# EndMy5uffering/4DGaussianSplatRendering

Hardware: AMD Instinct MI355X
Metric: Gaussians/sec + ms/frame @1080p; sort permutation bit-exact (higher is better)
Workload: dtype f32; 1 GPU; 1,000,000 random 3D splats in a 400^3 cube, single 1080p frame (BASELINE.json configs[1]); splats=1000000, width=1920, height=1080, sort=on, frame_lanes=4, tile_list_entries=1377553, longest_tile_list=477, unordered_draws=3158, staged_list_draws=3158, overflow_reruns=3, depth_sort_passes=3, record_bytes_read_by_projection=64, tiles_composited=14400, tiles=32400, key_index_buffer_pairs=4, lane_streams_rejected_at_create=1

## Files before the change

### 4dgaussiansplatrendering_amd/csrc/gs4d_internal.h

```cpp
#pragma once
#include <hip/hip_runtime.h>
#include <stdint.h>
#include <stddef.h>
#include <string>
#include <vector>
#include "../../include/gs4d.h"

namespace gs4d {

constexpr int TILE = 8;
constexpr int PROJ_FLOATS = 16;


enum class Outputs : int { Colour = 0, Aux = 1, Ids = 2 };
constexpr bool has_aux(Outputs o) { return o >= Outputs::Aux; }
constexpr bool has_ids(Outputs o) { return o >= Outputs::Ids; }
static_assert(sizeof(gs4d_record_stat) == 16 && offsetof(gs4d_record_stat, wsum) == 8, "the 64-bit sum is naturally aligned in a 16-byte record");
struct StatOut { gs4d_record_stat* rec = nullptr; uint32_t n = 0; };
struct Target {
    float4* fb; uint32_t* tstate; uint32_t epoch; float4 clear;
    Outputs out; float2* aux; uint32_t* ids;
    const float* z = nullptr;
    StatOut stats;
};
// ... 182 lines not shown
    TRect r{ tx0, ty0, wx, ty1 - ty0 + 1u, 1u, 0u };
    if (shard_world > 1u) {
        const uint32_t first = r.ty0 + (shard_rank + shard_world - r.ty0 % shard_world) % shard_world;
        r.rows = first > ty1 ? 0u : (ty1 - first) / shard_world + 1u;
        r.ty0 = first; r.tstep = shard_world;
    }
    r.count = r.wx * r.rows;
    return r;
}
__device__ __forceinline__ TRect tile_rect(uint32_t rect0, uint32_t rect1, uint32_t shard_rank, uint32_t shard_world) {
    const uint32_t x0 = rect0 & 0xFFFFu, y0 = rect0 >> 16, x1 = rect1 & 0xFFFFu, y1 = rect1 >> 16;
    if (x0 > x1 || y0 > y1) return TRect{ 0u, 0u, 0u, 0u, 1u, 0u };
    return tile_rect_of(x0 / TILE, y0 / TILE, x1 / TILE - x0 / TILE + 1u, y1 / TILE, shard_rank, shard_world);
}
constexpr uint32_t TRECT_NONE = 0xFFFFFFFFu, TRECT_WIDE = 0xFFFFFFFEu;
__device__ __forceinline__ uint32_t pack_trect(uint32_t rect0, uint32_t rect1) {
    const uint32_t x0 = rect0 & 0xFFFFu, y0 = rect0 >> 16, x1 = rect1 & 0xFFFFu, y1 = rect1 >> 16;
    if (x0 > x1 || y0 > y1) return TRECT_NONE;
    const uint32_t tx0 = x0 / TILE, ty0 = y0 / TILE, wx = x1 / TILE - tx0, wy = y1 / TILE - ty0;
    if (tx0 >= 1023u || ty0 >= 1023u || wx >= 63u || wy >= 63u) return TRECT_WIDE;
    return tx0 | (ty0 << 10) | (wx << 20) | (wy << 26);
}
__device__ __forceinline__ TRect unpack_trect(uint32_t w, const float4* __restrict__ proj, uint32_t rec, uint32_t shard_rank, uint32_t shard_world) {
    if (w == TRECT_NONE) return TRect{ 0u, 0u, 0u, 0u, 1u, 0u };
    if (w == TRECT_WIDE) { const float4 c = proj[(size_t)rec * 4 + 2]; return tile_rect(__float_as_uint(c.z), __float_as_uint(c.w), shard_rank, shard_world); }
    const uint32_t tx0 = w & 1023u, ty0 = (w >> 10) & 1023u;
    return tile_rect_of(tx0, ty0, ((w >> 20) & 63u) + 1u, ty0 + (w >> 26), shard_rank, shard_world);
}
__device__ __forceinline__ uint32_t tile_of(const TRect& r, uint32_t j, uint32_t tiles_x) { return (r.ty0 + (j / r.wx) * r.tstep) * tiles_x + r.tx0 + j % r.wx; }
template <class F> __device__ __forceinline__ void for_each_tile(const TRect& r, uint32_t tiles_x, F f) {
    uint32_t rowbase = r.ty0 * tiles_x + r.tx0;
    for (uint32_t y = 0; y < r.rows; ++y) { for (uint32_t x = 0; x < r.wx; ++x) f(rowbase + x); rowbase += r.tstep * tiles_x; }
}
#endif

hipError_t launch_soa_repack(hipStream_t st, const float* aos96, size_t n, float4* soa , uint32_t* bbox , const SoaInfo& info);
inline const float4* soa_sig3(const float4* soa, size_t n, const SoaInfo& info) { return info.layout == SOA_STATIC3D ? nullptr : soa + (info.layout == SOA_SYM ? 3 : 5) * n; }
struct PreOut { float4* proj; uint32_t* trects; bool aux = false; };
hipError_t launch_preprocess_4d(hipStream_t st, const float4* soa, size_t soa_n , const SoaInfo& info, size_t n, const Uniforms& u, int W, int H, PreOut out, const TileCount& tc);
hipError_t launch_preprocess_3d(hipStream_t st, const float* verts72, size_t n, const Uniforms& u, int W, int H, PreOut out, const TileCount& tc);
hipError_t launch_preprocess_2d(hipStream_t st, const float* rec48, size_t n, const Uniforms& u, int W, int H, PreOut out, const TileCount& tc);

struct BinScratch {
    uint32_t* total = nullptr;
    uint32_t* ranges = nullptr; size_t tiles_cap = 0;
    unsigned long long* status = nullptr; size_t block_cap = 0;
    uint32_t epoch = 0;
    uint32_t ticket_base = 0;
};
hipError_t bin_scratch_reserve(hipStream_t st, BinScratch& b, size_t ninst, size_t ntiles);
void bin_scratch_free(BinScratch& b);
hipError_t launch_binning(hipStream_t st, BinScratch& b, const uint32_t* trects, bool trects_in_order, const float4* proj, const uint32_t* order, uint32_t* order_copy, size_t ninst, size_t nrecords, int tiles_x, int tiles_y,
                          uint32_t* pair_keys, uint32_t* pair_vals, size_t pair_cap, uint32_t* err, uint32_t* ghist, int passes, uint32_t* total_host, int shard_rank, int shard_world);
hipError_t launch_tile_ranges(hipStream_t st, BinScratch& b, const uint32_t* pair_keys, size_t pair_cap, size_t ntiles);

hipError_t launch_composite(hipStream_t st, const float4* proj, const uint32_t* pair_vals, uint32_t* ranges, const uint32_t* total, int tiles_x, int tiles_y,
                            int W, int H, int premult_c, const Target& t, int blend_src, int blend_dst, uint32_t draw_ord);
hipError_t launch_fill_unwritten(hipStream_t st, const Target& t, int tiles_x, int tiles_y, int W, int H);
hipError_t launch_pack_rgba8(hipStream_t st, const float4* fb, const uint32_t* tstate, uint32_t epoch, const float clear[4], int W, int H, int tiles_x, uint32_t* out);
hipError_t launch_pack_rgba8_band(hipStream_t st, const float4* fb, const uint32_t* tstate, uint32_t epoch, const float clear[4], int W, int H, int tiles_x, int rank, int world, int band_rows, uint32_t* out);

struct LineParams { float vp[16]; float rgba[4]; int W, H; int blend_src, blend_dst; };
hipError_t launch_lines(hipStream_t st, const float* verts_dev, size_t nverts, int dims, int strip, const LineParams& p, float width, uint32_t* cnt, float4* fb);

constexpr uint32_t COMPACT_TILE = 2048;
struct KeepRule { uint32_t min_pixels, min_wmax; uint64_t min_wsum; uint32_t invert; };
// ... 97 lines not shown
```

### 4dgaussiansplatrendering_amd/csrc/preprocess.hip

```cpp
#include "gs4d_internal.h"
#include <algorithm>
#include <cstdlib>

namespace gs4d {

__device__ __forceinline__ uint32_t f2ord(float f) { const uint32_t u = __float_as_uint(f); return (u & 0x80000000u) ? ~u : (u | 0x80000000u); }

struct SoaConsts { float v[8]; };
template <int LAYOUT>
__global__ __launch_bounds__(256) void k_soa_repack(const float4* __restrict__ aos, uint32_t n, float4* __restrict__ soa, uint32_t* __restrict__ bbox, SoaConsts cs) {
    constexpr bool COMPACT = LAYOUT != SOA_FULL;
    __shared__ float4 stage[4][384];
    __shared__ uint32_t red[4][16];
    const uint32_t lane = threadIdx.x & 63u, w = threadIdx.x >> 6;
    uint32_t lo[7], hi[7];
#pragma unroll
    for (int k = 0; k < 7; ++k) { lo[k] = 0xFFFFFFFFu; hi[k] = 0u; }
    bool bad = false, asym = false;
    for (uint32_t chunk = blockIdx.x; chunk * 256u < n; chunk += gridDim.x) {
        const uint32_t rec0 = (chunk * 4u + w) * 64u;
        const uint32_t nrec = rec0 < n ? min(64u, n - rec0) : 0u;
#pragma unroll
        for (int j = 0; j < 6; ++j) {
            uint32_t f = j * 64u + lane;
// ... 32 lines not shown
        __builtin_amdgcn_wave_barrier();
    }
#pragma unroll
    for (int k = 0; k < 7; ++k) {
#pragma unroll
        for (int off = 32; off > 0; off >>= 1) { lo[k] = min(lo[k], (uint32_t)__shfl_xor(lo[k], off, 64)); hi[k] = max(hi[k], (uint32_t)__shfl_xor(hi[k], off, 64)); }
    }
    const bool anybad = __ballot(bad) != 0ull;
    if (COMPACT && __ballot(asym) != 0ull && lane == 0) atomicOr(&bbox[15], 1u);
    if (lane == 0) {
#pragma unroll
        for (int k = 0; k < 7; ++k) { red[w][k] = lo[k]; red[w][7 + k] = hi[k]; }
        red[w][14] = anybad ? 1u : 0u;
    }
    __syncthreads();
    if (threadIdx.x < 15u) {
        const uint32_t k = threadIdx.x;
        uint32_t v = red[0][k];
        for (int ww = 1; ww < 4; ++ww) v = k < 7u ? min(v, red[ww][k]) : k < 14u ? max(v, red[ww][k]) : (v | red[ww][k]);
        if (k < 7u) atomicMin(&bbox[k], v); else if (k < 14u) atomicMax(&bbox[k], v); else if (v) atomicOr(&bbox[14], 1u);
    }
}

hipError_t launch_soa_repack(hipStream_t st, const float* aos96, size_t n, float4* soa, uint32_t* bbox, const SoaInfo& info) {
    if (n == 0) return hipSuccess;
    const unsigned blocks = (unsigned)std::min<size_t>((n + 255) / 256, 2048);
    SoaConsts cs; for (int k = 0; k < 8; ++k) cs.v[k] = info.consts[k];
    if (info.layout == SOA_STATIC3D) k_soa_repack<SOA_STATIC3D><<<dim3(blocks), dim3(256), 0, st>>>((const float4*)aos96, (uint32_t)n, soa, bbox, cs);
    else if (info.layout == SOA_SYM) k_soa_repack<SOA_SYM><<<dim3(blocks), dim3(256), 0, st>>>((const float4*)aos96, (uint32_t)n, soa, bbox, cs);
    else k_soa_repack<SOA_FULL><<<dim3(blocks), dim3(256), 0, st>>>((const float4*)aos96, (uint32_t)n, soa, bbox, cs);
    return hipGetLastError();
}

struct PU { float V[16]; float P[16]; float time, min_opacity; int W, H; };

__device__ __forceinline__ float maxf_glsl(float a, float b) { return a >= b ? a : b; }
__device__ __forceinline__ void normalize2(float& x, float& y) { float tx = x * x, ty = y * y; float s = 1.0f / sqrtf(tx + ty); x = x * s; y = y * s; }

struct Quad { float e0x, e0y, e1x, e1y, s0, s1; };

__device__ __forceinline__ void eigen2(float u00, float u01, float u10, float u11, bool guard, float& lx, float& ly, Quad& q) {
    float m = (u00 + u11) * 0.5f;
    float p = (u00 * u11) - (u01 * u10);
    float d = sqrtf((m * m) - p);
    lx = maxf_glsl(m - d, 0.000001f);
    ly = maxf_glsl(m + d, 0.000001f);
    float ax, ay, bx, by;
    if (guard && u01 == 0.0f) { ax = 1.0f; ay = 0.0f; bx = 0.0f; by = 1.0f; }
    else {
        ax = u01; ay = lx - u00;
        normalize2(ax, ay);
        bx = ay; by = -ax;
        normalize2(ax, ay); normalize2(bx, by);
    }
    normalize2(ax, ay); normalize2(bx, by);
    q.e0x = ax; q.e0y = ay; q.e1x = bx; q.e1y = by;
}

__device__ __forceinline__ bool fin(float x) { return isfinite(x); }

__device__ __forceinline__ uint2 emit(const PreOut& out, uint32_t i, bool valid, const Quad& q, float ncx, float ncy, float kx, float ky,
                                      int W, int H, float r, float g, float b, float alpha, bool clamp_rgb, float depth) {
    float cx = 0, cy = 0, a0x = 0, a0y = 0, a1x = 0, a1y = 0, hx = 0, hy = 0;
    uint32_t rect0 = 1u, rect1 = 0u;
    if (valid) {
        float hw = (float)W * 0.5f, hh = (float)H * 0.5f;
        float sx = kx * hw, sy = ky * hh;
        cx = fmaf(ncx, hw, hw);
        cy = fmaf(ncy, hh, hh);
        float r0 = 1.0f / q.s0, r1 = 1.0f / q.s1;
        a0x = (q.e0x * r0) / sx; a0y = (q.e0y * r0) / sy;
        a1x = (q.e1x * r1) / sx; a1y = (q.e1y * r1) / sy;
        hx = 0.5f * (fabsf(q.e0x) * q.s0 + fabsf(q.e1x) * q.s1) * fabsf(sx);
        hy = 0.5f * (fabsf(q.e0y) * q.s0 + fabsf(q.e1y) * q.s1) * fabsf(sy);
        valid = fin(cx) && fin(cy) && fin(a0x) && fin(a0y) && fin(a1x) && fin(a1y) && fin(hx) && fin(hy) && fin(alpha);
        if (valid) {
            float mx = 0.01f + 1e-5f * hx, my = 0.01f + 1e-5f * hy;
            float fx0 = ceilf(cx - hx - mx - 0.5f), fx1 = floorf(cx + hx + mx - 0.5f);
            float fy0 = ceilf(cy - hy - my - 0.5f), fy1 = floorf(cy + hy + my - 0.5f);
            fx0 = fmaxf(fx0, 0.0f); fy0 = fmaxf(fy0, 0.0f);
            fx1 = fminf(fx1, (float)(W - 1)); fy1 = fminf(fy1, (float)(H - 1));
            if (fx0 <= fx1 && fy0 <= fy1) {
                rect0 = (uint32_t)fx0 | ((uint32_t)fy0 << 16);
                rect1 = (uint32_t)fx1 | ((uint32_t)fy1 << 16);
            }
        }
    }
    if (!valid) { cx = cy = a0x = a0y = a1x = a1y = hx = hy = 0.0f; alpha = 0.0f; rect0 = 1u; rect1 = 0u; depth = 0.0f; }
    if (clamp_rgb) { r = fminf(fmaxf(r, 0.0f), 1.0f); g = fminf(fmaxf(g, 0.0f), 1.0f); b = fminf(fmaxf(b, 0.0f), 1.0f); }
    if (out.trects) out.trects[i] = pack_trect(rect0, rect1);
    float4* o = out.proj + (size_t)i * 4;
    o[0] = make_float4(cx, cy, a0x, a1x);
    o[1] = make_float4(a0y, a1y, r, g);
    o[2] = make_float4(b, alpha, __uint_as_float(rect0), __uint_as_float(rect1));
    o[3] = make_float4(hx, hy, valid ? 1.0f : 0.0f, out.aux ? depth : 0.0f);
    return make_uint2(rect0, rect1);
}

__device__ __forceinline__ void count_buckets(uint32_t* h, uint32_t nbm, uint32_t tiles_x, const TRect& r) {
    const bool big = r.count > 16u;
    if (!big) for_each_tile(r, tiles_x, [&](uint32_t t) { atomicAdd(&h[t & nbm], 1u); });
    uint64_t m = __ballot(big);
    const uint32_t lane = threadIdx.x & 63u;
    while (m) {
        const int src = __ffsll((long long)m) - 1;
        m &= m - 1ull;
        TRect rr;
        rr.tx0 = __shfl(r.tx0, src, 64); rr.ty0 = __shfl(r.ty0, src, 64); rr.wx = __shfl(r.wx, src, 64);
        rr.rows = __shfl(r.rows, src, 64); rr.tstep = __shfl(r.tstep, src, 64); rr.count = __shfl(r.count, src, 64);
        for (uint32_t j = lane; j < rr.count; j += 64u) atomicAdd(&h[tile_of(rr, j, tiles_x) & nbm], 1u);
    }
}

__device__ __forceinline__ void place_buckets(uint32_t* cur, uint32_t nbm, uint32_t nbs, uint32_t tiles_x, const TRect& r, uint32_t key, uint32_t rec, uint2* stage) {
    const bool big = r.count > 16u;
    if (!big) for_each_tile(r, tiles_x, [&](uint32_t t) { stage[atomicAdd(&cur[t & nbm], 1u)] = make_uint2(key, ((t >> nbs) << 24) | rec); });
    uint64_t m = __ballot(big);
    const uint32_t lane = threadIdx.x & 63u;
    while (m) {
        const int src = __ffsll((long long)m) - 1;
        m &= m - 1ull;
        TRect rr;
        rr.tx0 = __shfl(r.tx0, src, 64); rr.ty0 = __shfl(r.ty0, src, 64); rr.wx = __shfl(r.wx, src, 64);
        rr.rows = __shfl(r.rows, src, 64); rr.tstep = __shfl(r.tstep, src, 64); rr.count = __shfl(r.count, src, 64);
        const uint32_t key2 = __shfl(key, src, 64), rec2 = __shfl(rec, src, 64);
        for (uint32_t j = lane; j < rr.count; j += 64u) { const uint32_t t = tile_of(rr, j, tiles_x); stage[atomicAdd(&cur[t & nbm], 1u)] = make_uint2(key2, ((t >> nbs) << 24) | rec2); }
    }
}

__device__ __forceinline__ uint32_t blend_key_4d(const KeySrc& ks, uint32_t i, const float4& p, const float4& s) {
    if (ks.mode == KEYSRC_INDEX) return i;
    float key;
    if (ks.mode == KEYSRC_REF) {
        float ct = ks.t - p.w;
        float x = p.x + s.x * ct;
        float y = p.y + s.y * ct;
        float z = p.z + s.z * ct;
        float dx = x - ks.camx, dy = y - ks.camy, dz = z - ks.camz;
        key = 1.0f / sqrtf(dx * dx + dy * dy + dz * dz);
    } else {
        float k = (1.0f / s.w) * (ks.t - p.w);
        float x = p.x + k * s.x, y = p.y + k * s.y, z = p.z + k * s.z;
        float zv = ((ks.vr0 * x + ks.vr1 * y) + ks.vr2 * z) + ks.vr3;
        key = 1.0f / fmaxf(-zv, 1e-20f);
    }
    return __float_as_uint(key) - ks.bias;
}

__device__ __forceinline__ bool project3d(const PU& u, float mx, float my, float mz, const float C[3][3], Quad& q, float& ncx, float& ncy, float& depth) {
// ... 24 lines not shown
    float T[3][3], Tt[3][3], A[3][3], cov[3][3];
#pragma unroll
    for (int c = 0; c < 3; ++c)
#pragma unroll
        for (int r = 0; r < 3; ++r) T[c][r] = Wt[0][r] * J[c][0] + Wt[1][r] * J[c][1] + Wt[2][r] * J[c][2];
#pragma unroll
    for (int c = 0; c < 3; ++c)
#pragma unroll
        for (int r = 0; r < 3; ++r) Tt[c][r] = T[r][c];
#pragma unroll
    for (int c = 0; c < 3; ++c)
#pragma unroll
        for (int r = 0; r < 3; ++r) A[c][r] = Tt[0][r] * C[c][0] + Tt[1][r] * C[c][1] + Tt[2][r] * C[c][2];
#pragma unroll
    for (int c = 0; c < 2; ++c)
#pragma unroll
        for (int r = 0; r < 2; ++r) cov[c][r] = A[0][r] * T[c][0] + A[1][r] * T[c][1] + A[2][r] * T[c][2];
    float lx, ly;
    eigen2(cov[0][0], cov[0][1], cov[1][0], cov[1][1], false, lx, ly, q);
    q.s0 = sqrtf(lx); q.s1 = sqrtf(ly);
    ncx = psx; ncy = psy;
    return true;
}

struct Src4D { const float4* soa; uint32_t stride; };
struct Src4DSym { const float4* soa; uint32_t stride; };
struct Src4DStatic { const float4* soa; uint32_t stride; SoaConsts cs; };
struct Src3D { const float* verts; };
struct Src2D { const float* recs; };

__device__ __forceinline__ uint2 project_4d(const float4& pos, const float4& col, const float4& s0, const float4& s1, const float4& s2, const float4& s3,
                                            uint32_t i, const PU& u, const PreOut& out, const KeySrc& ks, uint32_t& key);
__device__ __forceinline__ uint2 project_record(const Src4D& src, uint32_t n, uint32_t i, const PU& u, const PreOut& out, const KeySrc& ks, uint32_t& key) {
    const float4* __restrict__ soa = src.soa;
    const size_t ps = src.stride;
    const float4 pos = soa[i], col = soa[ps + i];
    const float4 s0 = soa[2 * ps + i], s1 = soa[3 * ps + i], s2 = soa[4 * ps + i], s3 = soa[5 * ps + i];
    return project_4d(pos, col, s0, s1, s2, s3, i, u, out, ks, key);
}
__device__ __forceinline__ uint2 project_record(const Src4DSym& src, uint32_t n, uint32_t i, const PU& u, const PreOut& out, const KeySrc& ks, uint32_t& key) {
    const float4* __restrict__ soa = src.soa;
    const size_t ps = src.stride;
    const float4 pos = soa[i], col = soa[ps + i], U = soa[2 * ps + i], V = soa[3 * ps + i];
    const float2 W = reinterpret_cast<const float2*>(soa + 4 * ps)[i];
    return project_4d(pos, col, make_float4(U.x, U.y, U.z, V.x), make_float4(U.y, U.w, W.x, V.y), make_float4(U.z, W.x, W.y, V.z), V, i, u, out, ks, key);
}
__device__ __forceinline__ uint2 project_record(const Src4DStatic& src, uint32_t n, uint32_t i, const PU& u, const PreOut& out, const KeySrc& ks, uint32_t& key) {
    const float4* __restrict__ soa = src.soa;
    const size_t ps = src.stride;
    const float4 A = soa[i], col = soa[ps + i], B = soa[2 * ps + i], C = soa[3 * ps + i];
    const float* c = src.cs.v;
    return project_4d(make_float4(A.x, A.y, A.z, c[0]), col, make_float4(A.w, B.x, B.y, c[1]), make_float4(B.z, B.w, C.x, c[2]), make_float4(C.y, C.z, C.w, c[3]), make_float4(c[4], c[5], c[6], c[7]),
                      i, u, out, ks, key);
}
__device__ __forceinline__ uint2 project_4d(const float4& pos, const float4& col, const float4& s0, const float4& s1, const float4& s2, const float4& s3,
                                            uint32_t i, const PU& u, const PreOut& out, const KeySrc& ks, uint32_t& key) {
    float s44 = s3.w;
    float dt = u.time - pos.w;
    float ot = maxf_glsl(expf(-0.5f * dt * (1.0f / s44) * dt), u.min_opacity);
    float ax = s0.w, ay = s1.w, az = s2.w;
    float k = (1.0f / s44) * dt;
    float mx = pos.x + k * ax, my = pos.y + k * ay, mz = pos.z + k * az;
    float inv = 1.0f / s44;
    float tv[3] = { inv * s3.x, inv * s3.y, inv * s3.z };
    float a[3] = { ax, ay, az };
    float S[3][3] = { { s0.x, s0.y, s0.z }, { s1.x, s1.y, s1.z }, { s2.x, s2.y, s2.z } };
    float C[3][3];
#pragma unroll
    for (int c = 0; c < 3; ++c)
#pragma unroll
        for (int r = 0; r < 3; ++r) C[c][r] = S[c][r] - a[r] * tv[c];
    Quad q; float ncx = 0, ncy = 0, depth = 0;
    bool valid = project3d(u, mx, my, mz, C, q, ncx, ncy, depth);
    key = blend_key_4d(ks, i, pos, s3);
    return emit(out, i, valid, q, ncx, ncy, u.P[0], u.P[5], u.W, u.H, col.x, col.y, col.z, ot * col.w, true, depth);
}

__device__ __forceinline__ uint2 project_record(const Src3D& src, uint32_t, uint32_t i, const PU& u, const PreOut& out, const KeySrc&, uint32_t& key) {
    const float* v = src.verts + (size_t)72 * i;
    float C[3][3];
#pragma unroll
    for (int c = 0; c < 3; ++c)
#pragma unroll
        for (int r = 0; r < 3; ++r) C[c][r] = v[9 + 3 * c + r];
    Quad q; float ncx = 0, ncy = 0, depth = 0;
    bool valid = project3d(u, v[2], v[3], v[4], C, q, ncx, ncy, depth);
    key = i;
    return emit(out, i, valid, q, ncx, ncy, u.P[0], u.P[5], u.W, u.H, v[5], v[6], v[7], v[8], false, depth);
}

__device__ __forceinline__ uint2 project_record(const Src2D& src, uint32_t, uint32_t i, const PU& u, const PreOut& out, const KeySrc&, uint32_t& key) {
    const float* rec = src.recs + (size_t)12 * i;
    const float* P = u.P;
    float x = rec[0], y = rec[1];
    float psx = ((P[0] * x + P[4] * y) + P[8] * -1.0f) + P[12] * 1.0f;
    float psy = ((P[1] * x + P[5] * y) + P[9] * -1.0f) + P[13] * 1.0f;
    float psz = ((P[2] * x + P[6] * y) + P[10] * -1.0f) + P[14] * 1.0f;
    float psw = ((P[3] * x + P[7] * y) + P[11] * -1.0f) + P[15] * 1.0f;
    float rw = 1.0f / psw;
    psx = rw * psx; psy = rw * psy; psz = rw * psz; psw = rw * psw;
    Quad q; float lx, ly;
    eigen2(rec[8], rec[9], rec[10], rec[11], true, lx, ly, q);
    float l0 = sqrtf(lx * 2.0f), l1 = sqrtf(ly * 2.0f);
    q.s0 = l1; q.s1 = l0;
    float zc = -5.0f + psz, wc4 = 1.0f + psw;
    float clipw = P[11] * zc + P[15] * wc4;
    float clipz = P[10] * zc + P[14] * wc4;
    bool valid = (clipw > 0.0f) && !(clipz < -clipw || clipz > clipw);
    float kx = P[0] / clipw, ky = P[5] / clipw;
    key = i;
    return emit(out, i, valid, q, kx * psx, ky * psy, kx, ky, u.W, u.H, rec[4], rec[5], rec[6], rec[7], true, 0.0f);
}

template <class SRC>
__global__ __launch_bounds__(256) void k_preprocess(SRC src, uint32_t n, PU u, PreOut out, TileCount tc) {
    const uint32_t i = blockIdx.x * 256u + threadIdx.x;
    if (i >= n) return;
    uint32_t key;
    (void)project_record(src, n, i, u, out, tc.ks, key);
}

static_assert(SEGFEED_BLOCK == (uint32_t)(STAGE_R * SEG_THREADS) && SEG_THREADS / 64 == 8 && OS_MAX_PASSES == 4, "segment-fed keys: a block per staged segment; eight waves' counters, four of them in kh");
constexpr size_t SEGFEED_LDS = (4 * OS_MAX_BINS) * 4 + (size_t)SEGFEED_BLOCK * 8;
template <class SRC, bool FUSE_KEYS, int COUNT, bool SEGF = false>
__global__ __launch_bounds__(SEG_THREADS) void k_project_count(SRC src, uint32_t n, PU u, PreOut out, TileCount tc) {
    __shared__ uint32_t h[COUNT ? 1024 : 1];
    __shared__ uint32_t kh[FUSE_KEYS ? OS_MAX_PASSES : 1][OS_MAX_BINS];
    __shared__ uint32_t ws[SEG_THREADS / 64 + 1];
    extern __shared__ __attribute__((aligned(16))) uint2 stage[];
    static_assert(!SEGF || (FUSE_KEYS && COUNT == 2), "segment-fed keys come from the staged, fused projection");
    constexpr bool segf = SEGF;
    const uint32_t wave = (uint32_t)__builtin_amdgcn_readfirstlane((int)(threadIdx.x >> 6));
    uint32_t* const stage32 = reinterpret_cast<uint32_t*>(stage);
    auto wave_row = [&](uint32_t k) -> uint32_t* { return k < 4u ? kh[FUSE_KEYS ? k : 0] : stage32 + (k - 4u) * OS_MAX_BINS; };
    if (COUNT) for (uint32_t b = threadIdx.x; b < tc.nb; b += SEG_THREADS) h[b] = 0u;
    if (FUSE_KEYS && threadIdx.x < 256u) os_hist_clear(kh, threadIdx.x);
    if (segf) for (uint32_t q = threadIdx.x; q < 4u * OS_MAX_BINS; q += SEG_THREADS) stage32[q] = 0u;
    __syncthreads();
    const uint32_t i0 = blockIdx.x * tc.seg, i1 = min(n, i0 + tc.seg);
    uint32_t s_key[COUNT == 2 ? STAGE_R : 1], s_r0[COUNT == 2 ? STAGE_R : 1], s_r1[COUNT == 2 ? STAGE_R : 1];
#pragma unroll
    for (int q = 0; q < (COUNT == 2 ? STAGE_R : 1); ++q) { s_key[q] = 0u; s_r0[q] = 1u; s_r1[q] = 0u; }
    auto staged_first = [&](int it) -> uint32_t { return segf ? i0 + wave * (uint32_t)(STAGE_R * 64) + (uint32_t)it * 64u : i0 + (uint32_t)it * SEG_THREADS; };
    auto staged_lane = [&]() -> uint32_t { return segf ? (threadIdx.x & 63u) : threadIdx.x; };
    auto round = [&](uint32_t i, int it) {
        TRect r{ 0u, 0u, 0u, 0u, 1u, 0u };
        uint32_t key = 0u;
        if (i < i1) {
            const uint2 rect = project_record(src, n, i, u, out, tc.ks, key);
            if (COUNT) {
                if (!FUSE_KEYS && COUNT == 1) tc.skey[i] = key;
                r = tile_rect(rect.x, rect.y, (uint32_t)tc.shard_rank, (uint32_t)tc.shard_world);
                if (COUNT == 2) { s_key[it] = key; s_r0[it] = rect.x; s_r1[it] = rect.y; }
            }
            if (FUSE_KEYS) {
                if (segf) {
                    atomicAdd(&wave_row(wave)[(key >> tc.hist_top) & (OS_MAX_BINS - 1u)], 1u);
                } else {
                    tc.keys_out[i] = __uint_as_float(key + tc.ks.bias);
                    if (tc.idx_out) tc.idx_out[i] = i;
                }
                if (key > tc.span) __hip_atomic_store(tc.err, 2u, __ATOMIC_RELAXED, __HIP_MEMORY_SCOPE_SYSTEM);
            }
        }
        if (FUSE_KEYS && !segf) os_hist_add(kh, key, i < i1, tc.hist_rows, tc.hist_rb, tc.hist_top);
        if (COUNT) count_buckets(h, tc.nb - 1u, (uint32_t)tc.tiles_x, r);
    };
    if (COUNT == 2) {
#pragma unroll
        for (int it = 0; it < STAGE_R; ++it) { const uint32_t ib = staged_first(it); if (ib >= i1) break; round(ib + staged_lane(), it); }
    } else {
        for (uint32_t ib = i0; ib < i1; ib += SEG_THREADS) round(ib + threadIdx.x, 0);
    }
    __syncthreads();
    if (segf) {
        const uint32_t tid = threadIdx.x, lane = tid & 63u;
        uint32_t wo[SEG_THREADS / 64], cnt = 0;
#pragma unroll
        for (int k = 0; k < SEG_THREADS / 64; ++k) { wo[k] = cnt; cnt += wave_row((uint32_t)k)[tid]; }
        uint32_t inc = cnt;
#pragma unroll
        for (int off = 1; off < 64; off <<= 1) { const uint32_t v = __shfl_up(inc, off, 64); if (lane >= (unsigned)off) inc += v; }
        if (lane == 63u) ws[wave] = inc;
        __syncthreads();
        uint32_t first = inc - cnt;
#pragma unroll
        for (int k = 0; k < SEG_THREADS / 64; ++k) if ((unsigned)k < wave) first += ws[k];
#pragma unroll
        for (int k = 0; k < SEG_THREADS / 64; ++k) wave_row((uint32_t)k)[tid] = first + wo[k];
        tc.seg_runs[(size_t)tid * tc.rows + blockIdx.x] = cnt | (first << 12);
        if (cnt) atomicAdd(&tc.ghist[((size_t)(blockIdx.x % OS_REPL) * OS_MAX_PASSES + OS_TOP_ROW) * OS_MAX_BINS + tid], cnt);
        __syncthreads();
        uint2* const pairs = stage + (4 * OS_MAX_BINS * 4) / sizeof(uint2);
        uint32_t* const mine = wave_row(wave);
#pragma unroll
        for (int q = 0; q < STAGE_R; ++q) {
            const uint32_t i = staged_first(q) + lane;
            if (i < i1) pairs[atomicAdd(&mine[(s_key[q] >> tc.hist_top) & (OS_MAX_BINS - 1u)], 1u)] = make_uint2(s_key[q] + tc.ks.bias, i);
        }
        __syncthreads();
        uint4* __restrict__ dst = reinterpret_cast<uint4*>(tc.seg_pairs + (size_t)blockIdx.x * SEGFEED_BLOCK);
        const uint4* src4 = reinterpret_cast<const uint4*>(pairs);
        for (uint32_t k = tid; k < (i1 - i0 + 1u) / 2u; k += SEG_THREADS) dst[k] = src4[k];
    }
    if (COUNT) {
        const uint32_t tid = threadIdx.x, lane = tid & 63u, w = tid >> 6, b0 = 2u * tid;
        const uint32_t c0 = b0 < tc.nb ? h[b0] : 0u, c1 = b0 + 1u < tc.nb ? h[b0 + 1u] : 0u, sum = c0 + c1;
        uint32_t inc = sum;
#pragma unroll
        for (int off = 1; off < 64; off <<= 1) { const uint32_t v = __shfl_up(inc, off, 64); if (lane >= (unsigned)off) inc += v; }
        if (lane == 63u) ws[w] = inc;
        __syncthreads();
        uint32_t base = 0, total = 0;
#pragma unroll
        for (int k = 0; k < SEG_THREADS / 64; ++k) { const uint32_t v = ws[k]; if ((unsigned)k < w) base += v; total += v; }
        const uint32_t o0 = base + inc - sum, o1 = o0 + c0;
        if (b0 < tc.nb) tc.hist[(size_t)b0 * tc.rows + blockIdx.x] = c0;
        if (b0 + 1u < tc.nb) tc.hist[(size_t)(b0 + 1u) * tc.rows + blockIdx.x] = c1;
        if (tid == 0u) tc.sstat[blockIdx.x] = total;
        if (COUNT == 2) {
            if (b0 < tc.nb) { tc.offs[(size_t)b0 * tc.rows + blockIdx.x] = o0; h[b0] = o0; }
            if (b0 + 1u < tc.nb) { tc.offs[(size_t)(b0 + 1u) * tc.rows + blockIdx.x] = o1; h[b0 + 1u] = o1; }
            const bool fits = total <= tc.scap;
            if (!fits && tid == 0u) *tc.abort_word = tc.seq;
            __syncthreads();
            if (fits) {
                const uint32_t nbs = (uint32_t)__ffs((int)tc.nb) - 1u;
#pragma unroll
                for (int q = 0; q < STAGE_R; ++q) {
                    const uint32_t i = staged_first(q) + staged_lane();
                    if (staged_first(q) >= i1) break;
                    const TRect r = i < i1 ? tile_rect(s_r0[q], s_r1[q], (uint32_t)tc.shard_rank, (uint32_t)tc.shard_world) : TRect{ 0u, 0u, 0u, 0u, 1u, 0u };
                    place_buckets(h, tc.nb - 1u, nbs, (uint32_t)tc.tiles_x, r, s_key[q], i, stage);
                }
                __syncthreads();
                uint4* __restrict__ dst = reinterpret_cast<uint4*>(tc.stage_out + (size_t)blockIdx.x * tc.scap);
                const uint4* src4 = reinterpret_cast<const uint4*>(stage);
                for (uint32_t k = tid; k < (total + 1u) / 2u; k += SEG_THREADS) dst[k] = src4[k];
            }
        }
    }
    if (FUSE_KEYS && !segf && threadIdx.x < 256u) os_hist_flush(kh, tc.ghist, tc.hist_rows, threadIdx.x, tc.hist_top);
}

static PU make_pu(const Uniforms& un, int W, int H) {
    PU u;
    for (int i = 0; i < 16; ++i) { u.V[i] = un.view[i]; u.P[i] = un.proj[i]; }
    u.time = un.time; u.min_opacity = un.min_opacity; u.W = W; u.H = H;
    return u;
}

template <class SRC>
static hipError_t launch_pre(hipStream_t st, SRC src, size_t n, const Uniforms& un, int W, int H, PreOut out, const TileCount& tc) {
    if (n == 0) return hipSuccess;
    if (tc.hist && tc.stage_out && tc.keys_out && tc.seg_pairs) k_project_count<SRC, true, 2, true><<<dim3((unsigned)((n + tc.seg - 1) / tc.seg)), dim3(SEG_THREADS), std::max<size_t>((size_t)tc.scap * 8, SEGFEED_LDS), st>>>(src, (uint32_t)n, make_pu(un, W, H), out, tc);
    else if (tc.hist && tc.stage_out && tc.keys_out) k_project_count<SRC, true, 2><<<dim3((unsigned)((n + tc.seg - 1) / tc.seg)), dim3(SEG_THREADS), (size_t)tc.scap * 8, st>>>(src, (uint32_t)n, make_pu(un, W, H), out, tc);
    else if (tc.hist && tc.stage_out) k_project_count<SRC, false, 2><<<dim3((unsigned)((n + tc.seg - 1) / tc.seg)), dim3(SEG_THREADS), (size_t)tc.scap * 8, st>>>(src, (uint32_t)n, make_pu(un, W, H), out, tc);
    else if (tc.hist && tc.keys_out) k_project_count<SRC, true, 1><<<dim3((unsigned)((n + tc.seg - 1) / tc.seg)), dim3(SEG_THREADS), 0, st>>>(src, (uint32_t)n, make_pu(un, W, H), out, tc);
    else if (tc.hist) k_project_count<SRC, false, 1><<<dim3((unsigned)((n + tc.seg - 1) / tc.seg)), dim3(SEG_THREADS), 0, st>>>(src, (uint32_t)n, make_pu(un, W, H), out, tc);
    else if (tc.keys_out) {
        TileCount t2 = tc;
        t2.seg = (uint32_t)std::max<size_t>(4096, (((n + 2047) / 2048) + SEG_THREADS - 1) / SEG_THREADS * SEG_THREADS);
        k_project_count<SRC, true, 0><<<dim3((unsigned)((n + t2.seg - 1) / t2.seg)), dim3(SEG_THREADS), 0, st>>>(src, (uint32_t)n, make_pu(un, W, H), out, t2);
    }
    else k_preprocess<SRC><<<dim3((unsigned)((n + 255) / 256)), dim3(256), 0, st>>>(src, (uint32_t)n, make_pu(un, W, H), out, tc);
    return hipGetLastError();
}
hipError_t launch_preprocess_4d(hipStream_t st, const float4* soa, size_t soa_n, const SoaInfo& info, size_t n, const Uniforms& un, int W, int H, PreOut out, const TileCount& tc) {
    if (info.layout == SOA_STATIC3D) { Src4DStatic s{ soa, (uint32_t)soa_n, SoaConsts() }; for (int k = 0; k < 8; ++k) s.cs.v[k] = info.consts[k]; return launch_pre(st, s, n, un, W, H, out, tc); }
    return info.layout == SOA_SYM ? launch_pre(st, Src4DSym{ soa, (uint32_t)soa_n }, n, un, W, H, out, tc) : launch_pre(st, Src4D{ soa, (uint32_t)soa_n }, n, un, W, H, out, tc);
}
hipError_t launch_preprocess_3d(hipStream_t st, const float* verts72, size_t n, const Uniforms& un, int W, int H, PreOut out, const TileCount& tc) { return launch_pre(st, Src3D{ verts72 }, n, un, W, H, out, tc); }
hipError_t launch_preprocess_2d(hipStream_t st, const float* rec48, size_t n, const Uniforms& un, int W, int H, PreOut out, const TileCount& tc) { return launch_pre(st, Src2D{ rec48 }, n, un, W, H, out, tc); }

}
```

Baseline: 10.97 billion splats/s.

## Cut register pressure in project-count kernel via packed tile rects and late kernarg loads

Several changes aim to reduce VGPR/SGPR pressure in the fused projection/binning kernel. Per-round tile rects are packed into one 32-bit word instead of two, and wide rects are re-read from the projection buffer. Kernel arguments are pinned to scalar registers with empty asm constraints, and the tail reads TileCount fields late through the kernarg segment pointer. A branchless 2x2 tile path is added for small footprints. The aux depth select becomes a mask, and the per-tile rect output is disabled in the staged mode. These compiler-steering tricks are fragile, and the late kernarg read assumes a fixed argument layout.

```diff
diff --git a/4dgaussiansplatrendering_amd/csrc/gs4d_internal.h b/4dgaussiansplatrendering_amd/csrc/gs4d_internal.h
--- a/4dgaussiansplatrendering_amd/csrc/gs4d_internal.h
+++ b/4dgaussiansplatrendering_amd/csrc/gs4d_internal.h
@@ -238,6 +238,14 @@
     uint32_t rowbase = r.ty0 * tiles_x + r.tx0;
     for (uint32_t y = 0; y < r.rows; ++y) { for (uint32_t x = 0; x < r.wx; ++x) f(rowbase + x); rowbase += r.tstep * tiles_x; }
 }
+__device__ __forceinline__ bool trect_2x2(const TRect& r) { return r.wx <= 2u && r.rows <= 2u; }
+template <class F> __device__ __forceinline__ void for_each_tile_2x2(const TRect& r, uint32_t tiles_x, F f) {
+    const uint32_t t0 = __umul24(r.ty0, tiles_x) + r.tx0, below = t0 + __umul24(r.tstep, tiles_x);
+    if (r.count >= 1u) f(t0);
+    if (r.wx == 2u && r.count >= 2u) f(t0 + 1u);
+    if (r.rows == 2u) f(below);
+    if (r.count == 4u) f(below + 1u);
+}
 #endif
 
 hipError_t launch_soa_repack(hipStream_t st, const float* aos96, size_t n, float4* soa , uint32_t* bbox , const SoaInfo& info);
diff --git a/4dgaussiansplatrendering_amd/csrc/preprocess.hip b/4dgaussiansplatrendering_amd/csrc/preprocess.hip
--- a/4dgaussiansplatrendering_amd/csrc/preprocess.hip
+++ b/4dgaussiansplatrendering_amd/csrc/preprocess.hip
@@ -88,7 +88,7 @@
     return hipGetLastError();
 }
 
-struct PU { float V[16]; float P[16]; float time, min_opacity; int W, H; };
+struct PU { float V[16]; float P[16]; float time, min_opacity; int W, H; uint32_t depth_mask; };
 
 __device__ __forceinline__ float maxf_glsl(float a, float b) { return a >= b ? a : b; }
 __device__ __forceinline__ void normalize2(float& x, float& y) { float tx = x * x, ty = y * y; float s = 1.0f / sqrtf(tx + ty); x = x * s; y = y * s; }
@@ -116,7 +116,7 @@
 __device__ __forceinline__ bool fin(float x) { return isfinite(x); }
 
 __device__ __forceinline__ uint2 emit(const PreOut& out, uint32_t i, bool valid, const Quad& q, float ncx, float ncy, float kx, float ky,
-                                      int W, int H, float r, float g, float b, float alpha, bool clamp_rgb, float depth) {
+                                      int W, int H, float r, float g, float b, float alpha, bool clamp_rgb, float depth, uint32_t depth_mask) {
     float cx = 0, cy = 0, a0x = 0, a0y = 0, a1x = 0, a1y = 0, hx = 0, hy = 0;
     uint32_t rect0 = 1u, rect1 = 0u;
     if (valid) {
@@ -149,13 +149,15 @@
     o[0] = make_float4(cx, cy, a0x, a1x);
     o[1] = make_float4(a0y, a1y, r, g);
     o[2] = make_float4(b, alpha, __uint_as_float(rect0), __uint_as_float(rect1));
-    o[3] = make_float4(hx, hy, valid ? 1.0f : 0.0f, out.aux ? depth : 0.0f);
+    o[3] = make_float4(hx, hy, valid ? 1.0f : 0.0f, __uint_as_float(__float_as_uint(depth) & depth_mask));
     return make_uint2(rect0, rect1);
 }
 
 __device__ __forceinline__ void count_buckets(uint32_t* h, uint32_t nbm, uint32_t tiles_x, const TRect& r) {
     const bool big = r.count > 16u;
-    if (!big) for_each_tile(r, tiles_x, [&](uint32_t t) { atomicAdd(&h[t & nbm], 1u); });
+    auto count = [&](uint32_t t) { atomicAdd(&h[t & nbm], 1u); };
+    if (trect_2x2(r)) for_each_tile_2x2(r, tiles_x, count);
+    else if (!big) for_each_tile(r, tiles_x, count);
     uint64_t m = __ballot(big);
     const uint32_t lane = threadIdx.x & 63u;
     while (m) {
@@ -170,7 +172,9 @@
 
 __device__ __forceinline__ void place_buckets(uint32_t* cur, uint32_t nbm, uint32_t nbs, uint32_t tiles_x, const TRect& r, uint32_t key, uint32_t rec, uint2* stage) {
     const bool big = r.count > 16u;
-    if (!big) for_each_tile(r, tiles_x, [&](uint32_t t) { stage[atomicAdd(&cur[t & nbm], 1u)] = make_uint2(key, ((t >> nbs) << 24) | rec); });
+    auto place = [&](uint32_t t) { stage[atomicAdd(&cur[t & nbm], 1u)] = make_uint2(key, ((t >> nbs) << 24) | rec); };
+    if (trect_2x2(r)) for_each_tile_2x2(r, tiles_x, place);
+    else if (!big) for_each_tile(r, tiles_x, place);
     uint64_t m = __ballot(big);
     const uint32_t lane = threadIdx.x & 63u;
     while (m) {
@@ -261,23 +265,23 @@
 __device__ __forceinline__ uint2 project_4d(const float4& pos, const float4& col, const float4& s0, const float4& s1, const float4& s2, const float4& s3,
                                             uint32_t i, const PU& u, const PreOut& out, const KeySrc& ks, uint32_t& key);
 __device__ __forceinline__ uint2 project_record(const Src4D& src, uint32_t n, uint32_t i, const PU& u, const PreOut& out, const KeySrc& ks, uint32_t& key) {
-    const float4* __restrict__ soa = src.soa;
+    const float4* __restrict__ rec = src.soa + i;
     const size_t ps = src.stride;
-    const float4 pos = soa[i], col = soa[ps + i];
-    const float4 s0 = soa[2 * ps + i], s1 = soa[3 * ps + i], s2 = soa[4 * ps + i], s3 = soa[5 * ps + i];
+    const float4 pos = rec[0], col = rec[ps];
+    const float4 s0 = rec[2 * ps], s1 = rec[3 * ps], s2 = rec[4 * ps], s3 = rec[5 * ps];
     return project_4d(pos, col, s0, s1, s2, s3, i, u, out, ks, key);
 }
 __device__ __forceinline__ uint2 project_record(const Src4DSym& src, uint32_t n, uint32_t i, const PU& u, const PreOut& out, const KeySrc& ks, uint32_t& key) {
-    const float4* __restrict__ soa = src.soa;
+    const float4* __restrict__ rec = src.soa + i;
     const size_t ps = src.stride;
-    const float4 pos = soa[i], col = soa[ps + i], U = soa[2 * ps + i], V = soa[3 * ps + i];
-    const float2 W = reinterpret_cast<const float2*>(soa + 4 * ps)[i];
+    const float4 pos = rec[0], col = rec[ps], U = rec[2 * ps], V = rec[3 * ps];
+    const float2 W = reinterpret_cast<const float2*>(src.soa + 4 * ps)[i];
     return project_4d(pos, col, make_float4(U.x, U.y, U.z, V.x), make_float4(U.y, U.w, W.x, V.y), make_float4(U.z, W.x, W.y, V.z), V, i, u, out, ks, key);
 }
 __device__ __forceinline__ uint2 project_record(const Src4DStatic& src, uint32_t n, uint32_t i, const PU& u, const PreOut& out, const KeySrc& ks, uint32_t& key) {
-    const float4* __restrict__ soa = src.soa;
+    const float4* __restrict__ rec = src.soa + i;
     const size_t ps = src.stride;
-    const float4 A = soa[i], col = soa[ps + i], B = soa[2 * ps + i], C = soa[3 * ps + i];
+    const float4 A = rec[0], col = rec[ps], B = rec[2 * ps], C = rec[3 * ps];
     const float* c = src.cs.v;
     return project_4d(make_float4(A.x, A.y, A.z, c[0]), col, make_float4(A.w, B.x, B.y, c[1]), make_float4(B.z, B.w, C.x, c[2]), make_float4(C.y, C.z, C.w, c[3]), make_float4(c[4], c[5], c[6], c[7]),
                       i, u, out, ks, key);
@@ -302,7 +306,7 @@
     Quad q; float ncx = 0, ncy = 0, depth = 0;
     bool valid = project3d(u, mx, my, mz, C, q, ncx, ncy, depth);
     key = blend_key_4d(ks, i, pos, s3);
-    return emit(out, i, valid, q, ncx, ncy, u.P[0], u.P[5], u.W, u.H, col.x, col.y, col.z, ot * col.w, true, depth);
+    return emit(out, i, valid, q, ncx, ncy, u.P[0], u.P[5], u.W, u.H, col.x, col.y, col.z, ot * col.w, true, depth, u.depth_mask);
 }
 
 __device__ __forceinline__ uint2 project_record(const Src3D& src, uint32_t, uint32_t i, const PU& u, const PreOut& out, const KeySrc&, uint32_t& key) {
@@ -315,7 +319,7 @@
     Quad q; float ncx = 0, ncy = 0, depth = 0;
     bool valid = project3d(u, v[2], v[3], v[4], C, q, ncx, ncy, depth);
     key = i;
-    return emit(out, i, valid, q, ncx, ncy, u.P[0], u.P[5], u.W, u.H, v[5], v[6], v[7], v[8], false, depth);
+    return emit(out, i, valid, q, ncx, ncy, u.P[0], u.P[5], u.W, u.H, v[5], v[6], v[7], v[8], false, depth, u.depth_mask);
 }
 
 __device__ __forceinline__ uint2 project_record(const Src2D& src, uint32_t, uint32_t i, const PU& u, const PreOut& out, const KeySrc&, uint32_t& key) {
@@ -338,7 +342,7 @@
     bool valid = (clipw > 0.0f) && !(clipz < -clipw || clipz > clipw);
     float kx = P[0] / clipw, ky = P[5] / clipw;
     key = i;
-    return emit(out, i, valid, q, kx * psx, ky * psy, kx, ky, u.W, u.H, rec[4], rec[5], rec[6], rec[7], true, 0.0f);
+    return emit(out, i, valid, q, kx * psx, ky * psy, kx, ky, u.W, u.H, rec[4], rec[5], rec[6], rec[7], true, 0.0f, 0u);
 }
 
 template <class SRC>
@@ -351,8 +355,29 @@
 
 static_assert(SEGFEED_BLOCK == (uint32_t)(STAGE_R * SEG_THREADS) && SEG_THREADS / 64 == 8 && OS_MAX_PASSES == 4, "segment-fed keys: a block per staged segment; eight waves' counters, four of them in kh");
 constexpr size_t SEGFEED_LDS = (4 * OS_MAX_BINS) * 4 + (size_t)SEGFEED_BLOCK * 8;
+template <class SRC> struct ProjArgs { SRC src; uint32_t n; PU u; PreOut out; TileCount tc; };
+__device__ __forceinline__ uint32_t used_here(uint32_t v) { asm volatile("" : "+s"(v)); return v; }
+template <class T> __device__ __forceinline__ void held(T& v) { asm volatile("" : "+s"(v)); }
+template <class T, int N> __device__ __forceinline__ void held(T (&v)[N]) {
+#pragma unroll
+    for (int k = 0; k < N; ++k) held(v[k]);
+}
+__device__ __forceinline__ void held(Src4D& s) { held(s.soa); held(s.stride); }
+__device__ __forceinline__ void held(Src4DSym& s) { held(s.soa); held(s.stride); }
+__device__ __forceinline__ void held(Src4DStatic& s) { held(s.soa); held(s.stride); held(s.cs.v); }
+__device__ __forceinline__ void held(Src3D& s) { held(s.verts); }
+__device__ __forceinline__ void held(Src2D& s) { held(s.recs); }
+__device__ __forceinline__ void held(PU& u) { held(u.V); held(u.P); held(u.time); held(u.min_opacity); held(u.W); held(u.H); held(u.depth_mask); }
+__device__ __forceinline__ void held(KeySrc& k) { held(k.mode); held(k.t); held(k.camx); held(k.camy); held(k.camz); held(k.vr0); held(k.vr1); held(k.vr2); held(k.vr3); held(k.bias); }
+template <class A> using KernArg = const A __attribute__((address_space(4)));
+template <class A> __device__ __forceinline__ KernArg<A>* late_args() {
+    KernArg<A>* p = (KernArg<A>*)__builtin_amdgcn_kernarg_segment_ptr();
+    asm volatile("" : "+s"(p));
+    return p;
+}
 template <class SRC, bool FUSE_KEYS, int COUNT, bool SEGF = false>
 __global__ __launch_bounds__(SEG_THREADS) void k_project_count(SRC src, uint32_t n, PU u, PreOut out, TileCount tc) {
+    held(src); held(u); held(out.proj); held(out.trects); held(tc.ks);
     __shared__ uint32_t h[COUNT ? 1024 : 1];
     __shared__ uint32_t kh[FUSE_KEYS ? OS_MAX_PASSES : 1][OS_MAX_BINS];
     __shared__ uint32_t ws[SEG_THREADS / 64 + 1];
@@ -367,20 +392,21 @@
     if (segf) for (uint32_t q = threadIdx.x; q < 4u * OS_MAX_BINS; q += SEG_THREADS) stage32[q] = 0u;
     __syncthreads();
     const uint32_t i0 = blockIdx.x * tc.seg, i1 = min(n, i0 + tc.seg);
-    uint32_t s_key[COUNT == 2 ? STAGE_R : 1], s_r0[COUNT == 2 ? STAGE_R : 1], s_r1[COUNT == 2 ? STAGE_R : 1];
-#pragma unroll
-    for (int q = 0; q < (COUNT == 2 ? STAGE_R : 1); ++q) { s_key[q] = 0u; s_r0[q] = 1u; s_r1[q] = 0u; }
+    uint32_t s_key[COUNT == 2 ? STAGE_R : 1], s_tr[COUNT == 2 ? STAGE_R : 1];
+#pragma unroll
+    for (int q = 0; q < (COUNT == 2 ? STAGE_R : 1); ++q) { s_key[q] = 0u; s_tr[q] = TRECT_NONE; }
     auto staged_first = [&](int it) -> uint32_t { return segf ? i0 + wave * (uint32_t)(STAGE_R * 64) + (uint32_t)it * 64u : i0 + (uint32_t)it * SEG_THREADS; };
     auto staged_lane = [&]() -> uint32_t { return segf ? (threadIdx.x & 63u) : threadIdx.x; };
+    const PreOut po{ out.proj, COUNT == 2 ? nullptr : out.trects, out.aux };
     auto round = [&](uint32_t i, int it) {
         TRect r{ 0u, 0u, 0u, 0u, 1u, 0u };
         uint32_t key = 0u;
         if (i < i1) {
-            const uint2 rect = project_record(src, n, i, u, out, tc.ks, key);
+            const uint2 rect = project_record(src, n, i, u, po, tc.ks, key);
             if (COUNT) {
                 if (!FUSE_KEYS && COUNT == 1) tc.skey[i] = key;
-                r = tile_rect(rect.x, rect.y, (uint32_t)tc.shard_rank, (uint32_t)tc.shard_world);
-                if (COUNT == 2) { s_key[it] = key; s_r0[it] = rect.x; s_r1[it] = rect.y; }
+                r = tile_rect(rect.x, rect.y, used_here((uint32_t)tc.shard_rank), used_here((uint32_t)tc.shard_world));
+                if (COUNT == 2) { s_key[it] = key; s_tr[it] = pack_trect(rect.x, rect.y); }
             }
             if (FUSE_KEYS) {
                 if (segf) {
@@ -392,7 +418,7 @@
                 if (key > tc.span) __hip_atomic_store(tc.err, 2u, __ATOMIC_RELAXED, __HIP_MEMORY_SCOPE_SYSTEM);
             }
         }
-        if (FUSE_KEYS && !segf) os_hist_add(kh, key, i < i1, tc.hist_rows, tc.hist_rb, tc.hist_top);
+        if (FUSE_KEYS && !segf) os_hist_add(kh, key, i < i1, (int)used_here((uint32_t)tc.hist_rows), tc.hist_rb, (int)used_here((uint32_t)tc.hist_top));
         if (COUNT) count_buckets(h, tc.nb - 1u, (uint32_t)tc.tiles_x, r);
     };
     if (COUNT == 2) {
@@ -402,6 +428,8 @@
         for (uint32_t ib = i0; ib < i1; ib += SEG_THREADS) round(ib + threadIdx.x, 0);
     }
     __syncthreads();
+    const auto* const lt = &late_args<ProjArgs<SRC>>()->tc;
+    (void)lt;
     if (segf) {
         const uint32_t tid = threadIdx.x, lane = tid & 63u;
         uint32_t wo[SEG_THREADS / 64], cnt = 0;
@@ -417,8 +445,8 @@
         for (int k = 0; k < SEG_THREADS / 64; ++k) if ((unsigned)k < wave) first += ws[k];
 #pragma unroll
         for (int k = 0; k < SEG_THREADS / 64; ++k) wave_row((uint32_t)k)[tid] = first + wo[k];
-        tc.seg_runs[(size_t)tid * tc.rows + blockIdx.x] = cnt | (first << 12);
-        if (cnt) atomicAdd(&tc.ghist[((size_t)(blockIdx.x % OS_REPL) * OS_MAX_PASSES + OS_TOP_ROW) * OS_MAX_BINS + tid], cnt);
+        lt->seg_runs[(size_t)tid * lt->rows + blockIdx.x] = cnt | (first << 12);
+        if (cnt) atomicAdd(&lt->ghist[((size_t)(blockIdx.x % OS_REPL) * OS_MAX_PASSES + OS_TOP_ROW) * OS_MAX_BINS + tid], cnt);
         __syncthreads();
         uint2* const pairs = stage + (4 * OS_MAX_BINS * 4) / sizeof(uint2);
         uint32_t* const mine = wave_row(wave);
@@ -428,13 +456,13 @@
             if (i < i1) pairs[atomicAdd(&mine[(s_key[q] >> tc.hist_top) & (OS_MAX_BINS - 1u)], 1u)] = make_uint2(s_key[q] + tc.ks.bias, i);
         }
         __syncthreads();
-        uint4* __restrict__ dst = reinterpret_cast<uint4*>(tc.seg_pairs + (size_t)blockIdx.x * SEGFEED_BLOCK);
+        uint4* __restrict__ dst = reinterpret_cast<uint4*>(lt->seg_pairs + (size_t)blockIdx.x * SEGFEED_BLOCK);
         const uint4* src4 = reinterpret_cast<const uint4*>(pairs);
         for (uint32_t k = tid; k < (i1 - i0 + 1u) / 2u; k += SEG_THREADS) dst[k] = src4[k];
     }
     if (COUNT) {
         const uint32_t tid = threadIdx.x, lane = tid & 63u, w = tid >> 6, b0 = 2u * tid;
-        const uint32_t c0 = b0 < tc.nb ? h[b0] : 0u, c1 = b0 + 1u < tc.nb ? h[b0 + 1u] : 0u, sum = c0 + c1;
+        const uint32_t c0 = b0 < lt->nb ? h[b0] : 0u, c1 = b0 + 1u < lt->nb ? h[b0 + 1u] : 0u, sum = c0 + c1;
         uint32_t inc = sum;
 #pragma unroll
         for (int off = 1; off < 64; off <<= 1) { const uint32_t v = __shfl_up(inc, off, 64); if (lane >= (unsigned)off) inc += v; }
@@ -444,26 +472,26 @@
 #pragma unroll
         for (int k = 0; k < SEG_THREADS / 64; ++k) { const uint32_t v = ws[k]; if ((unsigned)k < w) base += v; total += v; }
         const uint32_t o0 = base + inc - sum, o1 = o0 + c0;
-        if (b0 < tc.nb) tc.hist[(size_t)b0 * tc.rows + blockIdx.x] = c0;
-        if (b0 + 1u < tc.nb) tc.hist[(size_t)(b0 + 1u) * tc.rows + blockIdx.x] = c1;
-        if (tid == 0u) tc.sstat[blockIdx.x] = total;
+        if (b0 < lt->nb) lt->hist[(size_t)b0 * lt->rows + blockIdx.x] = c0;
+        if (b0 + 1u < lt->nb) lt->hist[(size_t)(b0 + 1u) * lt->rows + blockIdx.x] = c1;
+        if (tid == 0u) lt->sstat[blockIdx.x] = total;
         if (COUNT == 2) {
-            if (b0 < tc.nb) { tc.offs[(size_t)b0 * tc.rows + blockIdx.x] = o0; h[b0] = o0; }
-            if (b0 + 1u < tc.nb) { tc.offs[(size_t)(b0 + 1u) * tc.rows + blockIdx.x] = o1; h[b0 + 1u] = o1; }
-            const bool fits = total <= tc.scap;
-            if (!fits && tid == 0u) *tc.abort_word = tc.seq;
+            if (b0 < lt->nb) { lt->offs[(size_t)b0 * lt->rows + blockIdx.x] = o0; h[b0] = o0; }
+            if (b0 + 1u < lt->nb) { lt->offs[(size_t)(b0 + 1u) * lt->rows + blockIdx.x] = o1; h[b0 + 1u] = o1; }
+            const bool fits = total <= lt->scap;
+            if (!fits && tid == 0u) *lt->abort_word = lt->seq;
             __syncthreads();
             if (fits) {
-                const uint32_t nbs = (uint32_t)__ffs((int)tc.nb) - 1u;
+                const uint32_t nbs = (uint32_t)__ffs((int)lt->nb) - 1u;
 #pragma unroll
                 for (int q = 0; q < STAGE_R; ++q) {
                     const uint32_t i = staged_first(q) + staged_lane();
                     if (staged_first(q) >= i1) break;
-                    const TRect r = i < i1 ? tile_rect(s_r0[q], s_r1[q], (uint32_t)tc.shard_rank, (uint32_t)tc.shard_world) : TRect{ 0u, 0u, 0u, 0u, 1u, 0u };
-                    place_buckets(h, tc.nb - 1u, nbs, (uint32_t)tc.tiles_x, r, s_key[q], i, stage);
+                    const TRect r = unpack_trect(s_tr[q], out.proj, i, used_here((uint32_t)lt->shard_rank), used_here((uint32_t)lt->shard_world));
+                    place_buckets(h, lt->nb - 1u, nbs, (uint32_t)lt->tiles_x, r, s_key[q], i, stage);
                 }
                 __syncthreads();
-                uint4* __restrict__ dst = reinterpret_cast<uint4*>(tc.stage_out + (size_t)blockIdx.x * tc.scap);
+                uint4* __restrict__ dst = reinterpret_cast<uint4*>(lt->stage_out + (size_t)blockIdx.x * lt->scap);
                 const uint4* src4 = reinterpret_cast<const uint4*>(stage);
                 for (uint32_t k = tid; k < (total + 1u) / 2u; k += SEG_THREADS) dst[k] = src4[k];
             }
@@ -472,27 +500,28 @@
     if (FUSE_KEYS && !segf && threadIdx.x < 256u) os_hist_flush(kh, tc.ghist, tc.hist_rows, threadIdx.x, tc.hist_top);
 }
 
-static PU make_pu(const Uniforms& un, int W, int H) {
+static PU make_pu(const Uniforms& un, int W, int H, bool aux) {
     PU u;
     for (int i = 0; i < 16; ++i) { u.V[i] = un.view[i]; u.P[i] = un.proj[i]; }
-    u.time = un.time; u.min_opacity = un.min_opacity; u.W = W; u.H = H;
+    u.time = un.time; u.min_opacity = un.min_opacity; u.W = W; u.H = H; u.depth_mask = aux ? 0xFFFFFFFFu : 0u;
     return u;
 }
 
 template <class SRC>
 static hipError_t launch_pre(hipStream_t st, SRC src, size_t n, const Uniforms& un, int W, int H, PreOut out, const TileCount& tc) {
     if (n == 0) return hipSuccess;
-    if (tc.hist && tc.stage_out && tc.keys_out && tc.seg_pairs) k_project_count<SRC, true, 2, true><<<dim3((unsigned)((n + tc.seg - 1) / tc.seg)), dim3(SEG_THREADS), std::max<size_t>((size_t)tc.scap * 8, SEGFEED_LDS), st>>>(src, (uint32_t)n, make_pu(un, W, H), out, tc);
-    else if (tc.hist && tc.stage_out && tc.keys_out) k_project_count<SRC, true, 2><<<dim3((unsigned)((n + tc.seg - 1) / tc.seg)), dim3(SEG_THREADS), (size_t)tc.scap * 8, st>>>(src, (uint32_t)n, make_pu(un, W, H), out, tc);
-    else if (tc.hist && tc.stage_out) k_project_count<SRC, false, 2><<<dim3((unsigned)((n + tc.seg - 1) / tc.seg)), dim3(SEG_THREADS), (size_t)tc.scap * 8, st>>>(src, (uint32_t)n, make_pu(un, W, H), out, tc);
-    else if (tc.hist && tc.keys_out) k_project_count<SRC, true, 1><<<dim3((unsigned)((n + tc.seg - 1) / tc.seg)), dim3(SEG_THREADS), 0, st>>>(src, (uint32_t)n, make_pu(un, W, H), out, tc);
-    else if (tc.hist) k_project_count<SRC, false, 1><<<dim3((unsigned)((n + tc.seg - 1) / tc.seg)), dim3(SEG_THREADS), 0, st>>>(src, (uint32_t)n, make_pu(un, W, H), out, tc);
+    if (tc.stage_out && out.trects) return hipErrorInvalidValue;
+    if (tc.hist && tc.stage_out && tc.keys_out && tc.seg_pairs) k_project_count<SRC, true, 2, true><<<dim3((unsigned)((n + tc.seg - 1) / tc.seg)), dim3(SEG_THREADS), std::max<size_t>((size_t)tc.scap * 8, SEGFEED_LDS), st>>>(src, (uint32_t)n, make_pu(un, W, H, out.aux), out, tc);
+    else if (tc.hist && tc.stage_out && tc.keys_out) k_project_count<SRC, true, 2><<<dim3((unsigned)((n + tc.seg - 1) / tc.seg)), dim3(SEG_THREADS), (size_t)tc.scap * 8, st>>>(src, (uint32_t)n, make_pu(un, W, H, out.aux), out, tc);
+    else if (tc.hist && tc.stage_out) k_project_count<SRC, false, 2><<<dim3((unsigned)((n + tc.seg - 1) / tc.seg)), dim3(SEG_THREADS), (size_t)tc.scap * 8, st>>>(src, (uint32_t)n, make_pu(un, W, H, out.aux), out, tc);
+    else if (tc.hist && tc.keys_out) k_project_count<SRC, true, 1><<<dim3((unsigned)((n + tc.seg - 1) / tc.seg)), dim3(SEG_THREADS), 0, st>>>(src, (uint32_t)n, make_pu(un, W, H, out.aux), out, tc);
+    else if (tc.hist) k_project_count<SRC, false, 1><<<dim3((unsigned)((n + tc.seg - 1) / tc.seg)), dim3(SEG_THREADS), 0, st>>>(src, (uint32_t)n, make_pu(un, W, H, out.aux), out, tc);
     else if (tc.keys_out) {
         TileCount t2 = tc;
         t2.seg = (uint32_t)std::max<size_t>(4096, (((n + 2047) / 2048) + SEG_THREADS - 1) / SEG_THREADS * SEG_THREADS);
-        k_project_count<SRC, true, 0><<<dim3((unsigned)((n + t2.seg - 1) / t2.seg)), dim3(SEG_THREADS), 0, st>>>(src, (uint32_t)n, make_pu(un, W, H), out, t2);
-    }
-    else k_preprocess<SRC><<<dim3((unsigned)((n + 255) / 256)), dim3(256), 0, st>>>(src, (uint32_t)n, make_pu(un, W, H), out, tc);
+        k_project_count<SRC, true, 0><<<dim3((unsigned)((n + t2.seg - 1) / t2.seg)), dim3(SEG_THREADS), 0, st>>>(src, (uint32_t)n, make_pu(un, W, H, out.aux), out, t2);
+    }
+    else k_preprocess<SRC><<<dim3((unsigned)((n + 255) / 256)), dim3(256), 0, st>>>(src, (uint32_t)n, make_pu(un, W, H, out.aux), out, tc);
     return hipGetLastError();
 }
 hipError_t launch_preprocess_4d(hipStream_t st, const float4* soa, size_t soa_n, const SoaInfo& info, size_t n, const Uniforms& un, int W, int H, PreOut out, const TileCount& tc) {
```

Result: no change. 11.00 billion splats/s, median of 5 (+0.3%).
